# 23skdu/longbow

Measured on AMD Instinct MI355X. Metric: k-NN queries/sec (batch=1024, k=100), 1Mx768 f32, higher is better.
Workload: dtype f32

## Files before the change

### longbow_amd/csrc/kernels_gemm.hip

```cpp
#include "lb_admit.h"

#include <cstdlib>

namespace lb {

constexpr int BM = 128;
constexpr int BN = 128;
constexpr int BK = 32;
constexpr int GEMM_THREADS = 256;

struct GemmArgs {
    const float *X;
    const float *norm2;
    const float *rnorm;
    int64_t row_begin, row_end;
    int D;
    const float *Q;
    int nq;
    const uint8_t *mask;
    const uint32_t *rowmap;
    CandState cs;
    int n_row_tiles, n_q_tiles;
    int boot;
};

__device__ __forceinline__ int swz_off(int row, int chunk)
{
    return row * BK + ((chunk ^ ((row >> 1) & 7)) << 2);
}

template <int MODE>
__device__ __forceinline__ f32x4 load_chunk(const float *base, int64_t row, int D, int k)
{
    f32x4 v = {0.f, 0.f, 0.f, 0.f};
    const float *p = base + row * (int64_t)D + k;
    if (MODE == 2) {
        v = *reinterpret_cast<const f32x4 *>(p);
    } else if (MODE == 1) {
        if (k < D) v = *reinterpret_cast<const f32x4 *>(p);
    } else {
        if (k + 0 < D) v.x = p[0];
        if (k + 1 < D) v.y = p[1];
        if (k + 2 < D) v.z = p[2];
        if (k + 3 < D) v.w = p[3];
    }
    return v;
}

template <int METRIC, int ALIGNED, int SPLIT = 0>
__global__ __launch_bounds__(GEMM_THREADS, 2) void gemm_filter_kernel(GemmArgs a)
{
    constexpr bool GLDS = ALIGNED == 2;
    const int b = blockIdx.x;
    const int xcd = b & 7;
    const int in_xcd = b >> 3;
    const int qt = in_xcd % a.n_q_tiles;
    const int rt = (in_xcd / a.n_q_tiles) * 8 + xcd;
    if (rt >= a.n_row_tiles) return;

    __shared__ __attribute__((aligned(16))) float lds_all[2 * 2 * BM * BK + BM + BM + BM / 4];
    float(*lds)[2][BM * BK] = reinterpret_cast<float(*)[2][BM * BK]>(lds_all);
    float *s_aux = lds_all + 2 * 2 * BM * BK;
    uint32_t *s_rowid = reinterpret_cast<uint32_t *>(s_aux + BM);
    uint8_t *s_vis = reinterpret_cast<uint8_t *>(s_rowid + BM);

    const int tid = threadIdx.x;
    const int lane = tid & 63;
    const int wave = tid >> 6;
    const int wr = wave >> 1, wc = wave & 1;
    const int l31 = lane & 31, h = lane >> 5;

    const int64_t row0 = a.row_begin + (int64_t)rt * BM;
    const int q0 = qt * BN;
    const int64_t last_row = a.row_end - 1;
    const int last_q = a.nq - 1;

    auto corpus_row = [&](int64_t pos) -> int64_t {
        if (pos > last_row) pos = last_row;
        return a.rowmap ? (int64_t)a.rowmap[pos] : pos;
    };
    const int64_t side_ri = corpus_row(row0 + (tid & (BM - 1)));

    int st_row[4], st_ch[4];
    int64_t st_xrow[4];
    int st_qrow[4];
#pragma unroll
    for (int i = 0; i < 4; i++) {
        int c = tid + GEMM_THREADS * i;
        st_row[i] = c >> 3;
        st_ch[i] = c & 7;
        st_xrow[i] = corpus_row(row0 + st_row[i]);
        int qr = q0 + st_row[i];
        st_qrow[i] = qr < last_q ? qr : last_q;
    }

    f32x16 acc[2][2];
#pragma unroll
    for (int i = 0; i < 2; i++)
#pragma unroll
        for (int j = 0; j < 2; j++)
#pragma unroll
            for (int r = 0; r < 16; r++) acc[i][j][r] = 0.f;

    const int nk = (a.D + BK - 1) / BK;
    f32x4 ra[4], rb[4];

    const float *gsrcA[4], *gsrcB[4];
    if (GLDS) {
#pragma unroll
        for (int i = 0; i < 4; i++) {
            const int j = wave * 4 + i;
            const int row = j * 8 + (lane >> 3);
            const int c = (lane & 7) ^ ((row >> 1) & 7);
            const int64_t xr = corpus_row(row0 + row);
            int qr = q0 + row;
            if (qr > last_q) qr = last_q;
            gsrcA[i] = a.X + xr * (int64_t)a.D + 4 * c;
            gsrcB[i] = a.Q + (int64_t)qr * a.D + 4 * c;
        }
    }
    auto glds_stage = [&](int stage, int k0) {
#pragma unroll
        for (int i = 0; i < 4; i++) {
            const int j = wave * 4 + i;
            __builtin_amdgcn_global_load_lds(
                (const __attribute__((address_space(1))) void *)(gsrcA[i] + k0),
                (__attribute__((address_space(3))) void *)(&lds[stage][0][j * 8 * BK]), 16, 0,
                2);
            __builtin_amdgcn_global_load_lds(
                (const __attribute__((address_space(1))) void *)(gsrcB[i] + k0),
                (__attribute__((address_space(3))) void *)(&lds[stage][1][j * 8 * BK]), 16, 0, 0);
        }
    };

    if (GLDS) glds_stage(0, 0);
    const float aux_r = side_aux<METRIC>(a.norm2, a.rnorm, side_ri);
    uint8_t side_vis = 1;
    if (a.mask) side_vis = a.mask[side_ri];
    uint64_t tau_raw[2];
#pragma unroll
    for (int tn = 0; tn < 2; tn++) {
        const int qj = q0 + wc * 64 + tn * 32 + l31;
        tau_raw[tn] = lane_tau(a.cs.tau, qj, a.nq, a.boot);
    }
    if (tid < BM) {
        s_aux[tid] = aux_r;
        s_vis[tid] = (row0 + tid <= last_row && side_vis) ? (uint8_t)1 : (uint8_t)0;
        s_rowid[tid] = (uint32_t)side_ri;
    }
    float tau_key[2];
    uint32_t tau_row[2];
#pragma unroll
    for (int tn = 0; tn < 2; tn++) {
        tau_key[tn] = tau_key_of(tau_raw[tn]);
        tau_row[tn] = entry_row(tau_raw[tn]);
    }
    if (!GLDS) {
#pragma unroll
        for (int i = 0; i < 4; i++) {
            ra[i] = load_chunk<ALIGNED>(a.X, st_xrow[i], a.D, st_ch[i] * 4);
            rb[i] = load_chunk<ALIGNED>(a.Q, st_qrow[i], a.D, st_ch[i] * 4);
        }
#pragma unroll
        for (int i = 0; i < 4; i++) {
            *reinterpret_cast<f32x4 *>(&lds[0][0][swz_off(st_row[i], st_ch[i])]) = ra[i];
            *reinterpret_cast<f32x4 *>(&lds[0][1][swz_off(st_row[i], st_ch[i])]) = rb[i];
        }
    }
    __syncthreads();

    for (int kt = 0; kt < nk; kt++) {
        const int cur = kt & 1;
        const bool has_next = kt + 1 < nk;
        if (has_next) {
            const int k0 = (kt + 1) * BK;
            if (GLDS) {
                glds_stage(cur ^ 1, k0);
            } else {
#pragma unroll
                for (int i = 0; i < 4; i++) {
                    ra[i] = load_chunk<ALIGNED>(a.X, st_xrow[i], a.D, k0 + st_ch[i] * 4);
                    rb[i] = load_chunk<ALIGNED>(a.Q, st_qrow[i], a.D, k0 + st_ch[i] * 4);
                }
            }
        }
        const float *As = lds[cur][0];
        const float *Bs = lds[cur][1];
        if (SPLIT == 2) {
#pragma unroll
            for (int ks = 0; ks < 2; ks++) {
                const int ch = 4 * ks + 2 * h;
                bf16x8 ah[2], al[2], bh[2], bl[2];
#pragma unroll
                for (int t = 0; t < 2; t++) {
                    const int ra_ = wr * 64 + t * 32 + l31, rb_ = wc * 64 + t * 32 + l31;
                    const f32x4 a0 = *reinterpret_cast<const f32x4 *>(&As[swz_off(ra_, ch)]), a1 = *reinterpret_cast<const f32x4 *>(&As[swz_off(ra_, ch + 1)]);
                    const f32x4 b0 = *reinterpret_cast<const f32x4 *>(&Bs[swz_off(rb_, ch)]), b1 = *reinterpret_cast<const f32x4 *>(&Bs[swz_off(rb_, ch + 1)]);
                    const float xa[8] = {a0.x, a0.y, a0.z, a0.w, a1.x, a1.y, a1.z, a1.w};
                    const float xb[8] = {b0.x, b0.y, b0.z, b0.w, b1.x, b1.y, b1.z, b1.w};
#pragma unroll
                    for (int i = 0; i < 8; i++) {
                        const __bf16 ha = (__bf16)xa[i], hb = (__bf16)xb[i];
                        ah[t][i] = ha;
                        al[t][i] = (__bf16)(xa[i] - (float)ha);
                        bh[t][i] = hb;
                        bl[t][i] = (__bf16)(xb[i] - (float)hb);
                    }
                }
#pragma unroll
                for (int tm = 0; tm < 2; tm++)
#pragma unroll
                    for (int tn = 0; tn < 2; tn++) {
                        acc[tm][tn] = __builtin_amdgcn_mfma_f32_32x32x16_bf16(al[tm], bh[tn], acc[tm][tn], 0, 0, 0);
                        acc[tm][tn] = __builtin_amdgcn_mfma_f32_32x32x16_bf16(ah[tm], bl[tn], acc[tm][tn], 0, 0, 0);
                        acc[tm][tn] = __builtin_amdgcn_mfma_f32_32x32x16_bf16(ah[tm], bh[tn], acc[tm][tn], 0, 0, 0);
                    }
            }
        } else if (SPLIT == 1) {
            bf16x8 ah[2][2], al[2][2], bh[2][2], bl[2][2];
            auto ldfrag = [&](int buf, int ks) {
                const int kb = 4 * ks + h;
#pragma unroll
                for (int t = 0; t < 2; t++) {
                    const int ra_ = wr * 64 + t * 32 + l31, rb_ = wc * 64 + t * 32 + l31;
                    ah[buf][t] = __builtin_bit_cast(bf16x8, *reinterpret_cast<const f32x4 *>(&As[swz_off(ra_, kb)]));
                    al[buf][t] = __builtin_bit_cast(bf16x8, *reinterpret_cast<const f32x4 *>(&As[swz_off(ra_, 2 + kb)]));
                    bh[buf][t] = __builtin_bit_cast(bf16x8, *reinterpret_cast<const f32x4 *>(&Bs[swz_off(rb_, kb)]));
                    bl[buf][t] = __builtin_bit_cast(bf16x8, *reinterpret_cast<const f32x4 *>(&Bs[swz_off(rb_, 2 + kb)]));
                }
            };
            ldfrag(0, 0);
#pragma unroll
            for (int ks = 0; ks < 2; ks++) {
                const int cb = ks & 1;
                if (ks < 1) ldfrag(cb ^ 1, ks + 1);
#pragma unroll
                for (int tm = 0; tm < 2; tm++)
#pragma unroll
                    for (int tn = 0; tn < 2; tn++) {
                        acc[tm][tn] = __builtin_amdgcn_mfma_f32_32x32x16_bf16(al[cb][tm], bh[cb][tn], acc[tm][tn], 0, 0, 0);
                        acc[tm][tn] = __builtin_amdgcn_mfma_f32_32x32x16_bf16(ah[cb][tm], bl[cb][tn], acc[tm][tn], 0, 0, 0);
                        acc[tm][tn] = __builtin_amdgcn_mfma_f32_32x32x16_bf16(ah[cb][tm], bh[cb][tn], acc[tm][tn], 0, 0, 0);
                    }
            }
        } else {
        f32x4 fa[2][2], fb[2][2];
#pragma unroll
        for (int t = 0; t < 2; t++) {
            fa[0][t] = *reinterpret_cast<const f32x4 *>(&As[swz_off(wr * 64 + t * 32 + l31, h)]);
            fb[0][t] = *reinterpret_cast<const f32x4 *>(&Bs[swz_off(wc * 64 + t * 32 + l31, h)]);
        }
#pragma unroll
        for (int s = 0; s < 4; s++) {
            const int cb = s & 1, nb = cb ^ 1;
            if (s < 3) {
                const int ch = 2 * (s + 1) + h;
#pragma unroll
                for (int t = 0; t < 2; t++) {
                    fa[nb][t] = *reinterpret_cast<const f32x4 *>(&As[swz_off(wr * 64 + t * 32 + l31, ch)]);
                    fb[nb][t] = *reinterpret_cast<const f32x4 *>(&Bs[swz_off(wc * 64 + t * 32 + l31, ch)]);
                }
            }
#pragma unroll
            for (int e = 0; e < 4; e++)
#pragma unroll
                for (int tm = 0; tm < 2; tm++)
#pragma unroll
                    for (int tn = 0; tn < 2; tn++)
                        acc[tm][tn] = __builtin_amdgcn_mfma_f32_32x32x2f32(fa[cb][tm][e], fb[cb][tn][e],
                                                                          acc[tm][tn], 0, 0, 0);
            if (!GLDS && s == 1 && has_next) {
                const int nxt = cur ^ 1;
#pragma unroll
                for (int i = 0; i < 4; i++) {
                    *reinterpret_cast<f32x4 *>(&lds[nxt][0][swz_off(st_row[i], st_ch[i])]) = ra[i];
                    *reinterpret_cast<f32x4 *>(&lds[nxt][1][swz_off(st_row[i], st_ch[i])]) = rb[i];
                }
            }
        }
        }
        __syncthreads();
    }

    float aux[2][4][4];
    uint32_t rid[2][4][4];
    uint32_t vbits = 0;
#pragma unroll
    for (int tm = 0; tm < 2; tm++)
#pragma unroll
        for (int g = 0; g < 4; g++)
            vbits |= tile_rows4(s_aux, s_rowid, s_vis, wr * 64 + tm * 32 + 8 * g + 4 * h, aux[tm][g], rid[tm][g]) << (tm * 16 + g * 4);
#pragma unroll
    for (int tn = 0; tn < 2; tn++) {
        const int qj = q0 + wc * 64 + tn * 32 + l31;
        const bool qok = qj < a.nq;
        uint64_t *list = a.cs.lists + (size_t)(qok ? qj : 0) * a.cs.cap;
        if (a.boot) {
            if (qok) {
#pragma unroll
                for (int tm = 0; tm < 2; tm++)
#pragma unroll
                    for (int g = 0; g < 4; g++) {
                        const int64_t rbase = row0 + wr * 64 + tm * 32 + 8 * g + 4 * h;
                        uint64_t ent[4];
#pragma unroll
                        for (int e = 0; e < 4; e++)
                            ent[e] = ((vbits >> (tm * 16 + g * 4 + e)) & 1u) ? pack_entry(cand_key<METRIC>(acc[tm][tn][4 * g + e], aux[tm][g][e]), rid[tm][g][e]) : kEntryMax;
                        uint64_t *dst = list + (rbase - a.row_begin);
                        if (rbase + 3 < a.row_end) {
                            typedef unsigned long long u64x2 __attribute__((ext_vector_type(2)));
                            u64x2 v0 = {ent[0], ent[1]}, v1 = {ent[2], ent[3]};
                            *reinterpret_cast<u64x2 *>(dst) = v0;
                            *reinterpret_cast<u64x2 *>(dst + 2) = v1;
                        } else {
#pragma unroll
                            for (int e = 0; e < 4; e++)
                                if (rbase + e < a.row_end) dst[e] = ent[e];
                        }
                    }
            }
            continue;
        }
        uint32_t bits = 0;
#pragma unroll
        for (int tm = 0; tm < 2; tm++)
#pragma unroll
            for (int g = 0; g < 4; g++)
#pragma unroll
                for (int e = 0; e < 4; e++)
                    bits |= admit_exact(cand_key<METRIC>(acc[tm][tn][4 * g + e], aux[tm][g][e]), rid[tm][g][e], tau_key[tn], tau_row[tn]) << (tm * 16 + g * 4 + e);
        bits &= vbits;
        if (bits) {
            uint32_t pos = atomicAdd(&a.cs.cnt[qj], (uint32_t)__builtin_popcount(bits));
#pragma unroll
            for (int tm = 0; tm < 2; tm++)
#pragma unroll
                for (int g = 0; g < 4; g++)
#pragma unroll
                    for (int e = 0; e < 4; e++)
                        if (bits & (1u << (tm * 16 + g * 4 + e))) {
                            const uint32_t ri = rid[tm][g][e];
                            if (pos < a.cs.cap) list[pos] = pack_entry(cand_key<METRIC>(acc[tm][tn][4 * g + e], aux[tm][g][e]), ri);
                            pos++;
                        }
        }
    }
}

__global__ __launch_bounds__(256) void split_bf16_kernel(const float *src, float *dst, int64_t n8)
{
    for (int64_t i = (int64_t)blockIdx.x * blockDim.x + threadIdx.x; i < n8; i += (int64_t)gridDim.x * blockDim.x) {
        bf16x8 hi, lo;
        split_bf16x8(*reinterpret_cast<const f32x4 *>(src + i * 8), *reinterpret_cast<const f32x4 *>(src + i * 8 + 4), hi, lo);
        const int64_t grp = i >> 1;
        const int kb = (int)(i & 1);
        char *g = reinterpret_cast<char *>(dst) + grp * 64;
        *reinterpret_cast<bf16x8 *>(g + kb * 16) = hi;
        *reinterpret_cast<bf16x8 *>(g + 32 + kb * 16) = lo;
    }
}

void launch_split_bf16(const float *src, float *dst, int64_t rows, int D, hipStream_t s)
{
    const int64_t n8 = rows * (int64_t)D / 8;
    if (n8 <= 0) return;
    int64_t blocks = (n8 + 255) / 256;
    if (blocks > 16384) blocks = 16384;
    hipLaunchKernelGGL(split_bf16_kernel, dim3((unsigned)blocks), dim3(256), 0, s, src, dst, n8);
}

void launch_gemm_filter(int metric, const float *X, const float *norm2, const float *rnorm,
                        int64_t row_begin, int64_t row_end, int D, const float *Q, int nq,
                        const uint8_t *mask, const uint32_t *rowmap, CandState cs, bool boot, int split,
                        hipStream_t s)
{
    if (row_end <= row_begin || nq <= 0) return;
    GemmArgs a;
    a.rowmap = rowmap;
    a.boot = boot ? 1 : 0;
    a.X = X; a.norm2 = norm2; a.rnorm = rnorm;
    a.row_begin = row_begin; a.row_end = row_end; a.D = D;
    a.Q = Q; a.nq = nq; a.mask = mask; a.cs = cs;
    a.n_row_tiles = (int)((row_end - row_begin + BM - 1) / BM);
    a.n_q_tiles = (nq + BN - 1) / BN;
    const int groups = (a.n_row_tiles + 7) / 8;
    dim3 grid((unsigned)(groups * 8 * a.n_q_tiles));
    const bool aligned = (D % 4 == 0) && ((reinterpret_cast<uintptr_t>(X) & 15) == 0) &&
                         ((reinterpret_cast<uintptr_t>(Q) & 15) == 0);
    const int mode = !aligned ? 0 : (D % BK == 0 ? 2 : 1);
    if (split == 1) {
        if (metric == METRIC_L2) hipLaunchKernelGGL((gemm_filter_kernel<METRIC_L2, 2, 1>), grid, dim3(GEMM_THREADS), 0, s, a);
        else if (metric == METRIC_COS) hipLaunchKernelGGL((gemm_filter_kernel<METRIC_COS, 2, 1>), grid, dim3(GEMM_THREADS), 0, s, a);
        else hipLaunchKernelGGL((gemm_filter_kernel<METRIC_DOT, 2, 1>), grid, dim3(GEMM_THREADS), 0, s, a);
        return;
    }
    if (split == 2) {
        if (metric == METRIC_L2) hipLaunchKernelGGL((gemm_filter_kernel<METRIC_L2, 2, 2>), grid, dim3(GEMM_THREADS), 0, s, a);
        else if (metric == METRIC_COS) hipLaunchKernelGGL((gemm_filter_kernel<METRIC_COS, 2, 2>), grid, dim3(GEMM_THREADS), 0, s, a);
        else hipLaunchKernelGGL((gemm_filter_kernel<METRIC_DOT, 2, 2>), grid, dim3(GEMM_THREADS), 0, s, a);
        return;
    }
#define LB_GEMM(M, AL) hipLaunchKernelGGL((gemm_filter_kernel<M, AL>), grid, dim3(GEMM_THREADS), 0, s, a)
#define LB_GEMM_M(M)                 \
    do {                             \
        if (mode == 2) LB_GEMM(M, 2); \
        else if (mode == 1) LB_GEMM(M, 1); \
        else LB_GEMM(M, 0);           \
    } while (0)
    if (metric == METRIC_L2) LB_GEMM_M(METRIC_L2);
    else if (metric == METRIC_COS) LB_GEMM_M(METRIC_COS);
    else LB_GEMM_M(METRIC_DOT);
#undef LB_GEMM_M
#undef LB_GEMM
}

}
```

Measured before the change: 84660.

## Software-pipeline fp32 MFMA loop with interleaved LDS-direct loads and sched barriers

For the GLDS fp32 path, the K loop is restructured to prefetch two stages ahead. The next stage's first LDS fragment is loaded right after the barrier, and the global-to-LDS load pieces are interleaved between MFMAs using explicit sched_group_barrier directives. The aim is to hide global load issue and LDS read latency behind the MFMA stream, with one barrier per K step. In exchange it adds hand-tuned scheduling that is fragile to compiler changes, and it relies on the overwritten stage having been fully consumed before the barrier.

```diff
diff --git a/longbow_amd/csrc/kernels_gemm.hip b/longbow_amd/csrc/kernels_gemm.hip
--- a/longbow_amd/csrc/kernels_gemm.hip
+++ b/longbow_amd/csrc/kernels_gemm.hip
@@ -119,19 +119,25 @@
             gsrcB[i] = a.Q + (int64_t)qr * a.D + 4 * c;
         }
     }
-    auto glds_stage = [&](int stage, int k0) {
-#pragma unroll
-        for (int i = 0; i < 4; i++) {
-            const int j = wave * 4 + i;
+    const int wave_u = __builtin_amdgcn_readfirstlane(wave);
+    auto glds_piece = [&](int p, int stage, int k0) {
+        const int i = p >> 1;
+        const int j = wave_u * 4 + i;
+        if ((p & 1) == 0)
             __builtin_amdgcn_global_load_lds(
                 (const __attribute__((address_space(1))) void *)(gsrcA[i] + k0),
                 (__attribute__((address_space(3))) void *)(&lds[stage][0][j * 8 * BK]), 16, 0,
                 2);
+        else
             __builtin_amdgcn_global_load_lds(
                 (const __attribute__((address_space(1))) void *)(gsrcB[i] + k0),
                 (__attribute__((address_space(3))) void *)(&lds[stage][1][j * 8 * BK]), 16, 0, 0);
-        }
     };
+    auto glds_stage = [&](int stage, int k0) {
+#pragma unroll
+        for (int p = 0; p < 8; p++) glds_piece(p, stage, k0);
+    };
+    constexpr bool WIDE = GLDS && SPLIT == 0;
 
     if (GLDS) glds_stage(0, 0);
     const float aux_r = side_aux<METRIC>(a.norm2, a.rnorm, side_ri);
@@ -169,117 +175,192 @@
     }
     __syncthreads();
 
-    for (int kt = 0; kt < nk; kt++) {
-        const int cur = kt & 1;
-        const bool has_next = kt + 1 < nk;
-        if (has_next) {
-            const int k0 = (kt + 1) * BK;
-            if (GLDS) {
-                glds_stage(cur ^ 1, k0);
+    if constexpr (WIDE) {
+        struct Frag {
+            f32x4 a[2], b[2];
+        };
+        auto ldfrag = [&](Frag &f, int stage, int s) {
+            const float *As = lds[stage][0];
+            const float *Bs = lds[stage][1];
+            const int ch = 2 * s + h;
+#pragma unroll
+            for (int t = 0; t < 2; t++) {
+                f.a[t] = *reinterpret_cast<const f32x4 *>(&As[swz_off(wr * 64 + t * 32 + l31, ch)]);
+                f.b[t] = *reinterpret_cast<const f32x4 *>(&Bs[swz_off(wc * 64 + t * 32 + l31, ch)]);
+            }
+        };
+        auto mfma16 = [&](const Frag &f) {
+#pragma unroll
+            for (int e = 0; e < 4; e++)
+#pragma unroll
+                for (int tm = 0; tm < 2; tm++)
+#pragma unroll
+                    for (int tn = 0; tn < 2; tn++)
+                        acc[tm][tn] = __builtin_amdgcn_mfma_f32_32x32x2f32(f.a[tm][e], f.b[tn][e], acc[tm][tn], 0, 0, 0);
+        };
+        Frag F0, F1;
+        auto steps012 = [&](int cur) {
+            ldfrag(F1, cur, 1);
+            mfma16(F0);
+            ldfrag(F0, cur, 2);
+            mfma16(F1);
+            ldfrag(F1, cur, 3);
+            mfma16(F0);
+#pragma unroll
+            for (int s = 0; s < 3; s++) {
+                __builtin_amdgcn_sched_group_barrier(0x008, 2, 0);
+                __builtin_amdgcn_sched_group_barrier(0x100, 4, 0);
+                __builtin_amdgcn_sched_group_barrier(0x008, 14, 0);
+            }
+            __builtin_amdgcn_sched_barrier(0);
+        };
+        ldfrag(F0, 0, 0);
+        if (nk > 1) glds_stage(1, BK);
+        int kt = 0;
+        for (; kt + 2 < nk; kt++) {
+            const int cur = kt & 1;
+            steps012(cur);
+            __syncthreads();
+            const int k0 = (kt + 2) * BK;
+            ldfrag(F0, cur ^ 1, 0);
+#pragma unroll
+            for (int p = 0; p < 8; p++) glds_piece(p, cur, k0);
+            mfma16(F1);
+            __builtin_amdgcn_sched_group_barrier(0x008, 2, 0);
+            __builtin_amdgcn_sched_group_barrier(0x100, 4, 0);
+#pragma unroll
+            for (int p = 0; p < 7; p++) {
+                __builtin_amdgcn_sched_group_barrier(0x020, 1, 0);
+                __builtin_amdgcn_sched_group_barrier(0x008, 2, 0);
+            }
+            __builtin_amdgcn_sched_group_barrier(0x020, 1, 0);
+        }
+        if (kt + 1 < nk) {
+            const int cur = kt & 1;
+            steps012(cur);
+            __syncthreads();
+            ldfrag(F0, cur ^ 1, 0);
+            mfma16(F1);
+            __builtin_amdgcn_sched_group_barrier(0x008, 2, 0);
+            __builtin_amdgcn_sched_group_barrier(0x100, 4, 0);
+            __builtin_amdgcn_sched_group_barrier(0x008, 14, 0);
+            kt++;
+        }
+        steps012(kt & 1);
+        mfma16(F1);
+    } else {
+        for (int kt = 0; kt < nk; kt++) {
+            const int cur = kt & 1;
+            const bool has_next = kt + 1 < nk;
+            if (has_next) {
+                const int k0 = (kt + 1) * BK;
+                if (GLDS) {
+                    glds_stage(cur ^ 1, k0);
+                } else {
+#pragma unroll
+                    for (int i = 0; i < 4; i++) {
+                        ra[i] = load_chunk<ALIGNED>(a.X, st_xrow[i], a.D, k0 + st_ch[i] * 4);
+                        rb[i] = load_chunk<ALIGNED>(a.Q, st_qrow[i], a.D, k0 + st_ch[i] * 4);
+                    }
+                }
+            }
+            const float *As = lds[cur][0];
+            const float *Bs = lds[cur][1];
+            if (SPLIT == 2) {
+#pragma unroll
+                for (int ks = 0; ks < 2; ks++) {
+                    const int ch = 4 * ks + 2 * h;
+                    bf16x8 ah[2], al[2], bh[2], bl[2];
+#pragma unroll
+                    for (int t = 0; t < 2; t++) {
+                        const int ra_ = wr * 64 + t * 32 + l31, rb_ = wc * 64 + t * 32 + l31;
+                        const f32x4 a0 = *reinterpret_cast<const f32x4 *>(&As[swz_off(ra_, ch)]), a1 = *reinterpret_cast<const f32x4 *>(&As[swz_off(ra_, ch + 1)]);
+                        const f32x4 b0 = *reinterpret_cast<const f32x4 *>(&Bs[swz_off(rb_, ch)]), b1 = *reinterpret_cast<const f32x4 *>(&Bs[swz_off(rb_, ch + 1)]);
+                        const float xa[8] = {a0.x, a0.y, a0.z, a0.w, a1.x, a1.y, a1.z, a1.w};
+                        const float xb[8] = {b0.x, b0.y, b0.z, b0.w, b1.x, b1.y, b1.z, b1.w};
+#pragma unroll
+                        for (int i = 0; i < 8; i++) {
+                            const __bf16 ha = (__bf16)xa[i], hb = (__bf16)xb[i];
+                            ah[t][i] = ha;
+                            al[t][i] = (__bf16)(xa[i] - (float)ha);
+                            bh[t][i] = hb;
+                            bl[t][i] = (__bf16)(xb[i] - (float)hb);
+                        }
+                    }
+#pragma unroll
+                    for (int tm = 0; tm < 2; tm++)
+#pragma unroll
+                        for (int tn = 0; tn < 2; tn++) {
+                            acc[tm][tn] = __builtin_amdgcn_mfma_f32_32x32x16_bf16(al[tm], bh[tn], acc[tm][tn], 0, 0, 0);
+                            acc[tm][tn] = __builtin_amdgcn_mfma_f32_32x32x16_bf16(ah[tm], bl[tn], acc[tm][tn], 0, 0, 0);
+                            acc[tm][tn] = __builtin_amdgcn_mfma_f32_32x32x16_bf16(ah[tm], bh[tn], acc[tm][tn], 0, 0, 0);
+                        }
+                }
+            } else if (SPLIT == 1) {
+                bf16x8 ah[2][2], al[2][2], bh[2][2], bl[2][2];
+                auto ldfrag = [&](int buf, int ks) {
+                    const int kb = 4 * ks + h;
+#pragma unroll
+                    for (int t = 0; t < 2; t++) {
+                        const int ra_ = wr * 64 + t * 32 + l31, rb_ = wc * 64 + t * 32 + l31;
+                        ah[buf][t] = __builtin_bit_cast(bf16x8, *reinterpret_cast<const f32x4 *>(&As[swz_off(ra_, kb)]));
+                        al[buf][t] = __builtin_bit_cast(bf16x8, *reinterpret_cast<const f32x4 *>(&As[swz_off(ra_, 2 + kb)]));
+                        bh[buf][t] = __builtin_bit_cast(bf16x8, *reinterpret_cast<const f32x4 *>(&Bs[swz_off(rb_, kb)]));
+                        bl[buf][t] = __builtin_bit_cast(bf16x8, *reinterpret_cast<const f32x4 *>(&Bs[swz_off(rb_, 2 + kb)]));
+                    }
+                };
+                ldfrag(0, 0);
+#pragma unroll
+                for (int ks = 0; ks < 2; ks++) {
+                    const int cb = ks & 1;
+                    if (ks < 1) ldfrag(cb ^ 1, ks + 1);
+#pragma unroll
+                    for (int tm = 0; tm < 2; tm++)
+#pragma unroll
+                        for (int tn = 0; tn < 2; tn++) {
+                            acc[tm][tn] = __builtin_amdgcn_mfma_f32_32x32x16_bf16(al[cb][tm], bh[cb][tn], acc[tm][tn], 0, 0, 0);
+                            acc[tm][tn] = __builtin_amdgcn_mfma_f32_32x32x16_bf16(ah[cb][tm], bl[cb][tn], acc[tm][tn], 0, 0, 0);
+                            acc[tm][tn] = __builtin_amdgcn_mfma_f32_32x32x16_bf16(ah[cb][tm], bh[cb][tn], acc[tm][tn], 0, 0, 0);
+                        }
+                }
             } else {
-#pragma unroll
-                for (int i = 0; i < 4; i++) {
-                    ra[i] = load_chunk<ALIGNED>(a.X, st_xrow[i], a.D, k0 + st_ch[i] * 4);
-                    rb[i] = load_chunk<ALIGNED>(a.Q, st_qrow[i], a.D, k0 + st_ch[i] * 4);
+                f32x4 fa[2][2], fb[2][2];
+#pragma unroll
+                for (int t = 0; t < 2; t++) {
+                    fa[0][t] = *reinterpret_cast<const f32x4 *>(&As[swz_off(wr * 64 + t * 32 + l31, h)]);
+                    fb[0][t] = *reinterpret_cast<const f32x4 *>(&Bs[swz_off(wc * 64 + t * 32 + l31, h)]);
                 }
-            }
-        }
-        const float *As = lds[cur][0];
-        const float *Bs = lds[cur][1];
-        if (SPLIT == 2) {
-#pragma unroll
-            for (int ks = 0; ks < 2; ks++) {
-                const int ch = 4 * ks + 2 * h;
-                bf16x8 ah[2], al[2], bh[2], bl[2];
-#pragma unroll
-                for (int t = 0; t < 2; t++) {
-                    const int ra_ = wr * 64 + t * 32 + l31, rb_ = wc * 64 + t * 32 + l31;
-                    const f32x4 a0 = *reinterpret_cast<const f32x4 *>(&As[swz_off(ra_, ch)]), a1 = *reinterpret_cast<const f32x4 *>(&As[swz_off(ra_, ch + 1)]);
-                    const f32x4 b0 = *reinterpret_cast<const f32x4 *>(&Bs[swz_off(rb_, ch)]), b1 = *reinterpret_cast<const f32x4 *>(&Bs[swz_off(rb_, ch + 1)]);
-                    const float xa[8] = {a0.x, a0.y, a0.z, a0.w, a1.x, a1.y, a1.z, a1.w};
-                    const float xb[8] = {b0.x, b0.y, b0.z, b0.w, b1.x, b1.y, b1.z, b1.w};
-#pragma unroll
-                    for (int i = 0; i < 8; i++) {
-                        const __bf16 ha = (__bf16)xa[i], hb = (__bf16)xb[i];
-                        ah[t][i] = ha;
-                        al[t][i] = (__bf16)(xa[i] - (float)ha);
-                        bh[t][i] = hb;
-                        bl[t][i] = (__bf16)(xb[i] - (float)hb);
+#pragma unroll
+                for (int s = 0; s < 4; s++) {
+                    const int cb = s & 1, nb = cb ^ 1;
+                    if (s < 3) {
+                        const int ch = 2 * (s + 1) + h;
+#pragma unroll
+                        for (int t = 0; t < 2; t++) {
+                            fa[nb][t] = *reinterpret_cast<const f32x4 *>(&As[swz_off(wr * 64 + t * 32 + l31, ch)]);
+                            fb[nb][t] = *reinterpret_cast<const f32x4 *>(&Bs[swz_off(wc * 64 + t * 32 + l31, ch)]);
+                        }
+                    }
+#pragma unroll
+                    for (int e = 0; e < 4; e++)
+#pragma unroll
+                        for (int tm = 0; tm < 2; tm++)
+#pragma unroll
+                            for (int tn = 0; tn < 2; tn++)
+                                acc[tm][tn] = __builtin_amdgcn_mfma_f32_32x32x2f32(fa[cb][tm][e], fb[cb][tn][e],
+                                                                                  acc[tm][tn], 0, 0, 0);
+                    if (!GLDS && s == 1 && has_next) {
+                        const int nxt = cur ^ 1;
+#pragma unroll
+                        for (int i = 0; i < 4; i++) {
+                            *reinterpret_cast<f32x4 *>(&lds[nxt][0][swz_off(st_row[i], st_ch[i])]) = ra[i];
+                            *reinterpret_cast<f32x4 *>(&lds[nxt][1][swz_off(st_row[i], st_ch[i])]) = rb[i];
+                        }
                     }
                 }
-#pragma unroll
-                for (int tm = 0; tm < 2; tm++)
-#pragma unroll
-                    for (int tn = 0; tn < 2; tn++) {
-                        acc[tm][tn] = __builtin_amdgcn_mfma_f32_32x32x16_bf16(al[tm], bh[tn], acc[tm][tn], 0, 0, 0);
-                        acc[tm][tn] = __builtin_amdgcn_mfma_f32_32x32x16_bf16(ah[tm], bl[tn], acc[tm][tn], 0, 0, 0);
-                        acc[tm][tn] = __builtin_amdgcn_mfma_f32_32x32x16_bf16(ah[tm], bh[tn], acc[tm][tn], 0, 0, 0);
-                    }
-            }
-        } else if (SPLIT == 1) {
-            bf16x8 ah[2][2], al[2][2], bh[2][2], bl[2][2];
-            auto ldfrag = [&](int buf, int ks) {
-                const int kb = 4 * ks + h;
-#pragma unroll
-                for (int t = 0; t < 2; t++) {
-                    const int ra_ = wr * 64 + t * 32 + l31, rb_ = wc * 64 + t * 32 + l31;
-                    ah[buf][t] = __builtin_bit_cast(bf16x8, *reinterpret_cast<const f32x4 *>(&As[swz_off(ra_, kb)]));
-                    al[buf][t] = __builtin_bit_cast(bf16x8, *reinterpret_cast<const f32x4 *>(&As[swz_off(ra_, 2 + kb)]));
-                    bh[buf][t] = __builtin_bit_cast(bf16x8, *reinterpret_cast<const f32x4 *>(&Bs[swz_off(rb_, kb)]));
-                    bl[buf][t] = __builtin_bit_cast(bf16x8, *reinterpret_cast<const f32x4 *>(&Bs[swz_off(rb_, 2 + kb)]));
-                }
-            };
-            ldfrag(0, 0);
-#pragma unroll
-            for (int ks = 0; ks < 2; ks++) {
-                const int cb = ks & 1;
-                if (ks < 1) ldfrag(cb ^ 1, ks + 1);
-#pragma unroll
-                for (int tm = 0; tm < 2; tm++)
-#pragma unroll
-                    for (int tn = 0; tn < 2; tn++) {
-                        acc[tm][tn] = __builtin_amdgcn_mfma_f32_32x32x16_bf16(al[cb][tm], bh[cb][tn], acc[tm][tn], 0, 0, 0);
-                        acc[tm][tn] = __builtin_amdgcn_mfma_f32_32x32x16_bf16(ah[cb][tm], bl[cb][tn], acc[tm][tn], 0, 0, 0);
-                        acc[tm][tn] = __builtin_amdgcn_mfma_f32_32x32x16_bf16(ah[cb][tm], bh[cb][tn], acc[tm][tn], 0, 0, 0);
-                    }
-            }
-        } else {
-        f32x4 fa[2][2], fb[2][2];
-#pragma unroll
-        for (int t = 0; t < 2; t++) {
-            fa[0][t] = *reinterpret_cast<const f32x4 *>(&As[swz_off(wr * 64 + t * 32 + l31, h)]);
-            fb[0][t] = *reinterpret_cast<const f32x4 *>(&Bs[swz_off(wc * 64 + t * 32 + l31, h)]);
-        }
-#pragma unroll
-        for (int s = 0; s < 4; s++) {
-            const int cb = s & 1, nb = cb ^ 1;
-            if (s < 3) {
-                const int ch = 2 * (s + 1) + h;
-#pragma unroll
-                for (int t = 0; t < 2; t++) {
-                    fa[nb][t] = *reinterpret_cast<const f32x4 *>(&As[swz_off(wr * 64 + t * 32 + l31, ch)]);
-                    fb[nb][t] = *reinterpret_cast<const f32x4 *>(&Bs[swz_off(wc * 64 + t * 32 + l31, ch)]);
-                }
-            }
-#pragma unroll
-            for (int e = 0; e < 4; e++)
-#pragma unroll
-                for (int tm = 0; tm < 2; tm++)
-#pragma unroll
-                    for (int tn = 0; tn < 2; tn++)
-                        acc[tm][tn] = __builtin_amdgcn_mfma_f32_32x32x2f32(fa[cb][tm][e], fb[cb][tn][e],
-                                                                          acc[tm][tn], 0, 0, 0);
-            if (!GLDS && s == 1 && has_next) {
-                const int nxt = cur ^ 1;
-#pragma unroll
-                for (int i = 0; i < 4; i++) {
-                    *reinterpret_cast<f32x4 *>(&lds[nxt][0][swz_off(st_row[i], st_ch[i])]) = ra[i];
-                    *reinterpret_cast<f32x4 *>(&lds[nxt][1][swz_off(st_row[i], st_ch[i])]) = rb[i];
-                }
-            }
-        }
-        }
-        __syncthreads();
+            }
+            __syncthreads();
+        }
     }
 
     float aux[2][4][4];
```

Result: faster. 87380, median of 6 (+3.2%).
